# CloudEngineHub/FairyGen

Hardware: AMD Instinct MI355X
Metric: decoded frames/sec (sec/clip in config), Wan2.2-TI2V-5B 704x1280x121 @ 5 steps (higher is better)
Workload: dtype bf16

## Files before the change

fairygen_amd/csrc/dit_elementwise.hip:

```cpp
#include "common.h"
#include "rmsnorm_rope_row.h"

#ifndef FG_ROW_MIN_WAVES
#define FG_ROW_MIN_WAVES 4
#endif
#define FG_ROW_BOUNDS __launch_bounds__(256, FG_ROW_MIN_WAVES)

namespace {

__device__ __forceinline__ void row_moments(const Row& r, int C, int lane, float eps, float& mean, float& rstd) {
    const int nvec = C >> 3;
    float s = 0.f;
#pragma unroll
    for (int i = 0; i < kMaxVec; ++i)
#pragma unroll
        for (int j = 0; j < 8; ++j) s += r.v[i][j];
    mean = wave_sum(s) / (float)C;
    float q = 0.f;
#pragma unroll
    for (int i = 0; i < kMaxVec; ++i) {
        if (lane + i * 64 < nvec) {
#pragma unroll
            for (int j = 0; j < 8; ++j) {
                const float d = r.v[i][j] - mean;
                q += d * d;
            }
        }
    }
    const float var = wave_sum(q) / (float)C;
    rstd = 1.0f / sqrtf(var + eps);
}

__device__ __forceinline__ int64_t mod_row(int64_t row, int64_t mod_rows, int64_t first_rows) {
    return mod_rows == 1 ? 0 : (mod_rows == 2 ? (row < first_rows ? 0 : 1) : row);
}

template <int MODE>
__device__ __forceinline__ void norm_store(const Row& r, int C, int lane, float eps, const bf16* p0, const bf16* p1,
                                           bf16* out) {
    const int nvec = C >> 3;
    float mean, rstd;
    row_moments(r, C, lane, eps, mean, rstd);
#pragma unroll
    for (int i = 0; i < kMaxVec; ++i) {
        const int vi = lane + i * 64;
        if (vi < nvec) {
            const bf16x8 a = ld8(p0 + (int64_t)vi * 8);
            const bf16x8 b = ld8(p1 + (int64_t)vi * 8);
            float o[8];
#pragma unroll
            for (int j = 0; j < 8; ++j) {
                const float n = (r.v[i][j] - mean) * rstd;
                if (MODE == 0) {
                    const float y = rbf(n);
                    const float s1 = rbf(1.0f + (float)b[j]);
                    o[j] = rbf(y * s1) + (float)a[j];
                } else {
                    o[j] = n * (float)a[j] + (float)b[j];
                }
            }
            st8(out + (int64_t)vi * 8, o);
        }
    }
}

__device__ __forceinline__ uint32_t cvt2_fp8(float a, float b) {
    return (uint32_t)__builtin_amdgcn_cvt_pk_fp8_f32(a, b, 0, false) & 0xffffu;
}

template <int MODE, bool DUAL = false>
__device__ __forceinline__ void norm_store_fp8(Row& r, int C, int lane, float eps, const bf16* p0, const bf16* p1,
                                               uint8_t* out8, float* scale_out, float fp8_max, bf16* out16 = nullptr) {
    const int nvec = C >> 3;
    float mean, rstd;
    row_moments(r, C, lane, eps, mean, rstd);
    float amax = 0.f;
#pragma unroll
    for (int i = 0; i < kMaxVec; ++i) {
        const int vi = lane + i * 64;
        if (vi < nvec) {
            const bf16x8 a = ld8(p0 + (int64_t)vi * 8);
            const bf16x8 b = ld8(p1 + (int64_t)vi * 8);
#pragma unroll
            for (int j = 0; j < 8; ++j) {
                const float n = (r.v[i][j] - mean) * rstd;
                float o;
                if (MODE == 0) {
                    const float y = rbf(n);
                    const float s1 = rbf(1.0f + (float)b[j]);
                    o = rbf(y * s1) + (float)a[j];
                } else {
                    o = n * (float)a[j] + (float)b[j];
                }
                r.v[i][j] = rbf(o);
                amax = fmaxf(amax, fabsf(r.v[i][j]));
            }
            if (DUAL) st8(out16 + (int64_t)vi * 8, r.v[i]);
        }
    }
    amax = wave_max(amax);
    const float sc = fmaxf(rbf(amax / fp8_max), 1.0f);
    const float denom = sc + 1e-8f;
    if (lane == 0) *scale_out = sc;
#pragma unroll
    for (int i = 0; i < kMaxVec; ++i) {
        const int vi = lane + i * 64;
        if (vi < nvec) {
            u32x2 w;
// ... 26 lines not shown
    const int64_t row = (int64_t)blockIdx.x * kRowsPerBlock + (threadIdx.x >> 6);
    if (row >= rows) return;
    Row r;
    load_row(x + row * C, C, lane, r);
    const int64_t m = MODE == 0 ? mod_row(row, mod_rows, first_rows) : 0;
    norm_store_fp8<MODE, true>(r, C, lane, eps, p0 + m * mod_ld, p1 + m * mod_ld, out8 + row * C, scale_out + row, fp8_max, out + row * C);
}

__global__ FG_ROW_BOUNDS void ln_modulate_kernel(const bf16* __restrict__ x, const bf16* __restrict__ shift,
                                                          const bf16* __restrict__ scale, bf16* __restrict__ out,
                                                          int64_t rows, int C, float eps, int64_t mod_rows,
                                                          int64_t first_rows, int64_t mod_ld) {
    const int lane = threadIdx.x & 63;
    const int64_t row = (int64_t)blockIdx.x * kRowsPerBlock + (threadIdx.x >> 6);
    if (row >= rows) return;
    Row r;
    load_row(x + row * C, C, lane, r);
    const int64_t m = mod_row(row, mod_rows, first_rows);
    norm_store<0>(r, C, lane, eps, shift + m * mod_ld, scale + m * mod_ld, out + row * C);
}

__global__ FG_ROW_BOUNDS void ln_affine_kernel(const bf16* __restrict__ x, const bf16* __restrict__ w,
                                                        const bf16* __restrict__ b, bf16* __restrict__ out,
                                                        int64_t rows, int C, float eps) {
    const int lane = threadIdx.x & 63;
    const int64_t row = (int64_t)blockIdx.x * kRowsPerBlock + (threadIdx.x >> 6);
    if (row >= rows) return;
    Row r;
    load_row(x + row * C, C, lane, r);
    norm_store<1>(r, C, lane, eps, w, b, out + row * C);
}

template <int MODE>
__global__ FG_ROW_BOUNDS void residual_kernel(const bf16* __restrict__ x, const bf16* __restrict__ y,
                                                       const bf16* __restrict__ gate, bf16* __restrict__ x_out,
                                                       const bf16* __restrict__ p0, const bf16* __restrict__ p1,
                                                       bf16* __restrict__ norm_out, int64_t rows, int C, float eps,
                                                       int64_t mod_rows, int64_t first_rows, int64_t mod_ld,
                                                       uint8_t* __restrict__ norm_fp8 = nullptr, float* __restrict__ norm_scale = nullptr,
                                                       float fp8_max = 0.f) {
    const int lane = threadIdx.x & 63;
    const int64_t row = (int64_t)blockIdx.x * kRowsPerBlock + (threadIdx.x >> 6);
    if (row >= rows) return;
    const int nvec = C >> 3;
    const int64_t m = mod_row(row, mod_rows, first_rows);
    Row r;
#pragma unroll
    for (int i = 0; i < kMaxVec; ++i) {
        const int vi = lane + i * 64;
        if (vi < nvec) {
            const bf16x8 xv = ld8(x + row * C + (int64_t)vi * 8);
            const bf16x8 yv = ld8(y + row * C + (int64_t)vi * 8);
            if (gate != nullptr) {
                const bf16x8 gv = ld8(gate + m * mod_ld + (int64_t)vi * 8);
#pragma unroll
                for (int j = 0; j < 8; ++j) r.v[i][j] = rbf((float)xv[j] + rbf((float)gv[j] * (float)yv[j]));
            } else {
#pragma unroll
                for (int j = 0; j < 8; ++j) r.v[i][j] = rbf((float)xv[j] + (float)yv[j]);
            }
            st8(x_out + row * C + (int64_t)vi * 8, r.v[i]);
        } else {
#pragma unroll
            for (int j = 0; j < 8; ++j) r.v[i][j] = 0.f;
        }
    }
    if (norm_fp8 != nullptr) {
        if (MODE == 0) norm_store_fp8<0>(r, C, lane, eps, p0 + m * mod_ld, p1 + m * mod_ld, norm_fp8 + row * C, norm_scale + row, fp8_max);
        if (MODE == 1) norm_store_fp8<1>(r, C, lane, eps, p0, p1, norm_fp8 + row * C, norm_scale + row, fp8_max);
        return;
    }
    if (MODE == 0) norm_store<0>(r, C, lane, eps, p0 + m * mod_ld, p1 + m * mod_ld, norm_out + row * C);
    if (MODE == 1) norm_store<1>(r, C, lane, eps, p0, p1, norm_out + row * C);
}

template <bool F32TAB, bool PLAIN = false>
__global__ FG_ROW_BOUNDS void rmsnorm_rope_kernel(const bf16* __restrict__ x, int64_t ldx,
                                                           const bf16* __restrict__ w, const void* __restrict__ ctv,
                                                           const void* __restrict__ stv, bf16* __restrict__ out,
                                                           int64_t rows, int C, int head_dim, float eps, int group_cols,
                                                           int64_t out_group_stride, int64_t out_ld) {
    const int lane = threadIdx.x & 63;
    const int64_t row = (int64_t)blockIdx.x * kRowsPerBlock + (threadIdx.x >> 6);
    if (row >= rows) return;
    Row r;
    load_row(x + row * ldx, C, lane, r);
    const int nvec = C >> 3;
    const RopeRow rr = rope_begin<F32TAB, PLAIN>(r, ctv, row, C, head_dim, eps, lane);
#pragma unroll
    for (int i = 0; i < kMaxVec; ++i) {
        const int vi = lane + i * 64;
        if (vi < nvec) {
            float o[8];
            rope_vec<F32TAB, PLAIN>(rr, r.v[i], ld8(w + (int64_t)vi * 8), ctv, stv, row, head_dim, vi, o);
            const int col = vi * 8, g = PLAIN ? 0 : col / group_cols;
            st8(out + g * out_group_stride + row * out_ld + (col - g * group_cols), o);
        }
    }
}

__global__ __launch_bounds__(256) void copy_groups_kernel(const bf16* __restrict__ src, int64_t sgs, int64_t sld,
                                                          bf16* __restrict__ dst, int64_t dgs, int64_t dld, int groups,
                                                          int64_t rows, int vec_per_row) {
    const int64_t total = (int64_t)groups * rows * vec_per_row;
    for (int64_t i = (int64_t)blockIdx.x * blockDim.x + threadIdx.x; i < total; i += (int64_t)gridDim.x * blockDim.x) {
        const int64_t rg = i / vec_per_row;
        const int v = (int)(i - rg * vec_per_row);
        const int64_t r = rg / groups;
        const int g = (int)(rg - r * groups);
        *reinterpret_cast<u32x4*>(dst + g * dgs + r * dld + v * 8) =
            *reinterpret_cast<const u32x4*>(src + g * sgs + r * sld + v * 8);
    }
}


template <int KIND>
__global__ __launch_bounds__(256) void act_kernel(const bf16* __restrict__ x, bf16* __restrict__ out, int64_t nvec) {
    for (int64_t i = (int64_t)blockIdx.x * blockDim.x + threadIdx.x; i < nvec; i += (int64_t)gridDim.x * blockDim.x) {
        const bf16x8 v = ld8(x + i * 8);
        float o[8];
#pragma unroll
        for (int j = 0; j < 8; ++j) o[j] = KIND == 0 ? silu_f((float)v[j]) : gelu_tanh_f((float)v[j]);
        st8(out + i * 8, o);
    }
}

__device__ __forceinline__ float cfg_euler_one(float lat, float p, float ng, bool has_nega, float cfg, float dsigma) {
    const float pred = has_nega ? rbf(ng + rbf(cfg * rbf(p - ng))) : p;
    return rbf(lat + rbf(pred * dsigma));
// ... 22 lines not shown
        if (first != nullptr) {
            int64_t ch = (i * 8) / frame_stride, r = i * 8 - ch * frame_stride;
            if (r < first_n || r + 7 >= frame_stride) {
#pragma unroll
                for (int j = 0; j < 8; ++j) {
                    if (r < first_n) o[j] = (float)first[ch * first_n + r];
                    if (++r == frame_stride) { r = 0; ++ch; }
                }
            }
        }
        st8(out + i * 8, o);
    }
    for (int64_t i = nvec * 8 + tid; i < n; i += nthreads) {
        float o = cfg_euler_one((float)lat[i], (float)posi[i], has_nega ? (float)nega[i] : 0.0f, has_nega, cfg, dsigma);
        if (first != nullptr) {
            const int64_t ch = i / frame_stride, r = i - ch * frame_stride;
            if (r < first_n) o = (float)first[ch * first_n + r];
        }
        out[i] = (bf16)o;
    }
}

inline int check_rows(const char* fn, int64_t rows, int C, int64_t mod_rows, int64_t first_rows) {
    FG_CHECK_ARG(rows >= 0 && C > 0 && (C % 8) == 0 && C <= kMaxVec * 512, "%s: need C %% 8 == 0 and C <= %d (got rows=%lld C=%d)",
                 fn, kMaxVec * 512, (long long)rows, C);
    FG_CHECK_ARG(mod_rows == 1 || mod_rows == 2 || mod_rows == rows, "%s: mod_rows must be 1, 2 or rows (got %lld)", fn,
                 (long long)mod_rows);
    FG_CHECK_ARG(first_rows >= 0 && first_rows <= rows, "%s: first_rows out of range", fn);
    return FG_OK;
}

inline dim3 row_grid(int64_t rows) { return dim3((unsigned)((rows + kRowsPerBlock - 1) / kRowsPerBlock)); }

}

extern "C" {

int fg_ln_modulate_bf16(const void* x, const void* shift, const void* scale, void* out, int64_t rows, int C, float eps,
                        int64_t mod_rows, int64_t first_rows, int64_t mod_ld, fg_stream_t stream) {
    if (int e = check_rows("fg_ln_modulate_bf16", rows, C, mod_rows, first_rows)) return e;
    FG_CHECK_ARG(x && shift && scale && out, "fg_ln_modulate_bf16: null pointer");
    FG_CHECK_ARG(FG_ALIGNED16(x) && FG_ALIGNED16(shift) && FG_ALIGNED16(scale) && FG_ALIGNED16(out) && mod_ld % 8 == 0,
                 "fg_ln_modulate_bf16: pointers / mod_ld must be 16-byte aligned");
    if (rows == 0) return FG_OK;
    hipLaunchKernelGGL(ln_modulate_kernel, row_grid(rows), dim3(256), 0, (hipStream_t)stream, (const bf16*)x,
                       (const bf16*)shift, (const bf16*)scale, (bf16*)out, rows, C, eps, mod_rows, first_rows, mod_ld);
    return fg_launch_status("fg_ln_modulate_bf16");
}

int fg_ln_modulate_fp8_bf16(const void* x, const void* shift, const void* scale, void* out_fp8, float* out_scale, int64_t rows, int C,
                            float eps, int64_t mod_rows, int64_t first_rows, int64_t mod_ld, float fp8_max, fg_stream_t stream) {
    if (int e = check_rows("fg_ln_modulate_fp8_bf16", rows, C, mod_rows, first_rows)) return e;
    FG_CHECK_ARG(x && shift && scale && out_fp8 && out_scale, "fg_ln_modulate_fp8_bf16: null pointer");
    FG_CHECK_ARG(FG_ALIGNED16(x) && FG_ALIGNED16(shift) && FG_ALIGNED16(scale) && (((uintptr_t)out_fp8) & 7) == 0 && mod_ld % 8 == 0 &&
                     fp8_max > 0.f,
                 "fg_ln_modulate_fp8_bf16: pointers / mod_ld must be 16-byte aligned (out_fp8: 8), fp8_max positive");
    if (rows == 0) return FG_OK;
    hipLaunchKernelGGL(ln_modulate_fp8_kernel, row_grid(rows), dim3(256), 0, (hipStream_t)stream, (const bf16*)x, (const bf16*)shift,
                       (const bf16*)scale, (uint8_t*)out_fp8, out_scale, rows, C, eps, mod_rows, first_rows, mod_ld, fp8_max);
    return fg_launch_status("fg_ln_modulate_fp8_bf16");
}

int fg_ln_modulate_dual_bf16(const void* x, const void* shift, const void* scale, void* out, void* out_fp8, float* out_scale,
                             int64_t rows, int C, float eps, int64_t mod_rows, int64_t first_rows, int64_t mod_ld, float fp8_max,
                             fg_stream_t stream) {
    if (int e = check_rows("fg_ln_modulate_dual_bf16", rows, C, mod_rows, first_rows)) return e;
    FG_CHECK_ARG(x && shift && scale && out && out_fp8 && out_scale, "fg_ln_modulate_dual_bf16: null pointer");
    FG_CHECK_ARG(FG_ALIGNED16(x) && FG_ALIGNED16(shift) && FG_ALIGNED16(scale) && FG_ALIGNED16(out) && (((uintptr_t)out_fp8) & 7) == 0 &&
                     mod_ld % 8 == 0 && fp8_max > 0.f,
                 "fg_ln_modulate_dual_bf16: pointers / mod_ld must be 16-byte aligned (out_fp8: 8), fp8_max positive");
    if (rows == 0) return FG_OK;
    hipLaunchKernelGGL(ln_dual_kernel<0>, row_grid(rows), dim3(256), 0, (hipStream_t)stream, (const bf16*)x, (const bf16*)shift,
                       (const bf16*)scale, (bf16*)out, (uint8_t*)out_fp8, out_scale, rows, C, eps, mod_rows, first_rows, mod_ld, fp8_max);
    return fg_launch_status("fg_ln_modulate_dual_bf16");
}

int fg_ln_affine_dual_bf16(const void* x, const void* w, const void* b, void* out, void* out_fp8, float* out_scale, int64_t rows, int C,
                           float eps, float fp8_max, fg_stream_t stream) {
    if (int e = check_rows("fg_ln_affine_dual_bf16", rows, C, 1, 0)) return e;
    FG_CHECK_ARG(x && w && b && out && out_fp8 && out_scale, "fg_ln_affine_dual_bf16: null pointer");
// ... 1 lines not shown
                     fp8_max > 0.f,
                 "fg_ln_affine_dual_bf16: pointers must be 16-byte aligned (out_fp8: 8), fp8_max positive");
    if (rows == 0) return FG_OK;
    hipLaunchKernelGGL(ln_dual_kernel<1>, row_grid(rows), dim3(256), 0, (hipStream_t)stream, (const bf16*)x, (const bf16*)w,
                       (const bf16*)b, (bf16*)out, (uint8_t*)out_fp8, out_scale, rows, C, eps, (int64_t)1, (int64_t)0, (int64_t)0, fp8_max);
    return fg_launch_status("fg_ln_affine_dual_bf16");
}

int fg_residual_ln_fp8_bf16(const void* x, const void* y, const void* gate, void* x_out, const void* p0, const void* p1,
                            void* norm_fp8, float* norm_scale, int mode, int64_t rows, int C, float eps, int64_t mod_rows,
                            int64_t first_rows, int64_t mod_ld, float fp8_max, fg_stream_t stream) {
    FG_CHECK_ARG(mode == 0 || mode == 1, "fg_residual_ln_fp8_bf16: mode must be 0 (modulate) or 1 (affine)");
    const bool need_mod = gate != nullptr || mode == 0;
    if (int e = check_rows("fg_residual_ln_fp8_bf16", rows, C, need_mod ? mod_rows : 1, need_mod ? first_rows : 0)) return e;
    FG_CHECK_ARG(x && y && x_out && p0 && p1 && norm_fp8 && norm_scale, "fg_residual_ln_fp8_bf16: null pointer");
    FG_CHECK_ARG(FG_ALIGNED16(x) && FG_ALIGNED16(y) && FG_ALIGNED16(gate) && FG_ALIGNED16(x_out) && FG_ALIGNED16(p0) &&
                     FG_ALIGNED16(p1) && (((uintptr_t)norm_fp8) & 7) == 0 && mod_ld % 8 == 0 && fp8_max > 0.f,
                 "fg_residual_ln_fp8_bf16: pointers / mod_ld must be 16-byte aligned (norm_fp8: 8), fp8_max positive");
    if (rows == 0) return FG_OK;
    if (!need_mod) { mod_rows = 1; first_rows = 0; }
    if (mode == 0)
        hipLaunchKernelGGL(residual_kernel<0>, row_grid(rows), dim3(256), 0, (hipStream_t)stream, (const bf16*)x,
                           (const bf16*)y, (const bf16*)gate, (bf16*)x_out, (const bf16*)p0, (const bf16*)p1,
                           (bf16*)nullptr, rows, C, eps, mod_rows, first_rows, mod_ld, (uint8_t*)norm_fp8, norm_scale, fp8_max);
    else
        hipLaunchKernelGGL(residual_kernel<1>, row_grid(rows), dim3(256), 0, (hipStream_t)stream, (const bf16*)x,
                           (const bf16*)y, (const bf16*)gate, (bf16*)x_out, (const bf16*)p0, (const bf16*)p1,
                           (bf16*)nullptr, rows, C, eps, mod_rows, first_rows, mod_ld, (uint8_t*)norm_fp8, norm_scale, fp8_max);
    return fg_launch_status("fg_residual_ln_fp8_bf16");
}

int fg_ln_affine_bf16(const void* x, const void* w, const void* b, void* out, int64_t rows, int C, float eps,
                      fg_stream_t stream) {
    if (int e = check_rows("fg_ln_affine_bf16", rows, C, 1, 0)) return e;
    FG_CHECK_ARG(x && w && b && out, "fg_ln_affine_bf16: null pointer");
    FG_CHECK_ARG(FG_ALIGNED16(x) && FG_ALIGNED16(w) && FG_ALIGNED16(b) && FG_ALIGNED16(out),
                 "fg_ln_affine_bf16: pointers must be 16-byte aligned");
    if (rows == 0) return FG_OK;
    hipLaunchKernelGGL(ln_affine_kernel, row_grid(rows), dim3(256), 0, (hipStream_t)stream, (const bf16*)x, (const bf16*)w,
                       (const bf16*)b, (bf16*)out, rows, C, eps);
    return fg_launch_status("fg_ln_affine_bf16");
}

int fg_gate_residual_bf16(const void* x, const void* y, const void* gate, void* out, int64_t rows, int C, int64_t mod_rows,
                          int64_t first_rows, int64_t mod_ld, fg_stream_t stream) {
    if (int e = check_rows("fg_gate_residual_bf16", rows, C, gate ? mod_rows : 1, gate ? first_rows : 0)) return e;
    FG_CHECK_ARG(x && y && out, "fg_gate_residual_bf16: null pointer");
    FG_CHECK_ARG(FG_ALIGNED16(x) && FG_ALIGNED16(y) && FG_ALIGNED16(gate) && FG_ALIGNED16(out) && mod_ld % 8 == 0,
                 "fg_gate_residual_bf16: pointers / mod_ld must be 16-byte aligned");
    if (rows == 0) return FG_OK;
    hipLaunchKernelGGL(residual_kernel<-1>, row_grid(rows), dim3(256), 0, (hipStream_t)stream, (const bf16*)x,
                       (const bf16*)y, (const bf16*)gate, (bf16*)out, (const bf16*)nullptr, (const bf16*)nullptr,
                       (bf16*)nullptr, rows, C, 0.f, gate ? mod_rows : 1, gate ? first_rows : 0, mod_ld);
    return fg_launch_status("fg_gate_residual_bf16");
}

int fg_residual_ln_bf16(const void* x, const void* y, const void* gate, void* x_out, const void* p0, const void* p1,
                        void* norm_out, int mode, int64_t rows, int C, float eps, int64_t mod_rows, int64_t first_rows,
                        int64_t mod_ld, fg_stream_t stream) {
    FG_CHECK_ARG(mode == 0 || mode == 1, "fg_residual_ln_bf16: mode must be 0 (modulate) or 1 (affine)");
    const bool need_mod = gate != nullptr || mode == 0;
    if (int e = check_rows("fg_residual_ln_bf16", rows, C, need_mod ? mod_rows : 1, need_mod ? first_rows : 0)) return e;
    FG_CHECK_ARG(x && y && x_out && p0 && p1 && norm_out, "fg_residual_ln_bf16: null pointer");
    FG_CHECK_ARG(FG_ALIGNED16(x) && FG_ALIGNED16(y) && FG_ALIGNED16(gate) && FG_ALIGNED16(x_out) && FG_ALIGNED16(p0) &&
                     FG_ALIGNED16(p1) && FG_ALIGNED16(norm_out) && mod_ld % 8 == 0,
                 "fg_residual_ln_bf16: pointers / mod_ld must be 16-byte aligned");
    if (rows == 0) return FG_OK;
    if (!need_mod) { mod_rows = 1; first_rows = 0; }
    if (mode == 0)
        hipLaunchKernelGGL(residual_kernel<0>, row_grid(rows), dim3(256), 0, (hipStream_t)stream, (const bf16*)x,
                           (const bf16*)y, (const bf16*)gate, (bf16*)x_out, (const bf16*)p0, (const bf16*)p1,
                           (bf16*)norm_out, rows, C, eps, mod_rows, first_rows, mod_ld);
    else
        hipLaunchKernelGGL(residual_kernel<1>, row_grid(rows), dim3(256), 0, (hipStream_t)stream, (const bf16*)x,
                           (const bf16*)y, (const bf16*)gate, (bf16*)x_out, (const bf16*)p0, (const bf16*)p1,
                           (bf16*)norm_out, rows, C, eps, mod_rows, first_rows, mod_ld);
    return fg_launch_status("fg_residual_ln_bf16");
}

int fg_rmsnorm_rope_bf16(const void* x, int64_t ldx, const void* weight, const void* cos_tab, const void* sin_tab,
                         int table_f32, void* out, int64_t rows, int C, int num_heads, float eps, fg_stream_t stream) {
    if (int e = check_rows("fg_rmsnorm_rope_bf16", rows, C, 1, 0)) return e;
    FG_CHECK_ARG(x && weight && out, "fg_rmsnorm_rope_bf16: null pointer");
    FG_CHECK_ARG(table_f32 ? (cos_tab != nullptr && sin_tab == nullptr) : ((cos_tab == nullptr) == (sin_tab == nullptr)),
                 "fg_rmsnorm_rope_bf16: fp64 mode takes both tables or neither, fp32 mode ONE interleaved table in cos_tab");
    FG_CHECK_ARG(num_heads > 0 && C % num_heads == 0 && (C / num_heads) % 8 == 0,
                 "fg_rmsnorm_rope_bf16: head_dim must be a multiple of 8");
    FG_CHECK_ARG(ldx >= C && ldx % 8 == 0 && FG_ALIGNED16(x) && FG_ALIGNED16(weight) && FG_ALIGNED16(out) &&
                     FG_ALIGNED16(cos_tab) && FG_ALIGNED16(sin_tab),
                 "fg_rmsnorm_rope_bf16: pointers / ldx must be 16-byte aligned");
    if (rows == 0) return FG_OK;
    const int hd = C / num_heads;
    const bool plain = (hd & (hd - 1)) == 0;
#define FG_ROPE_LAUNCH(TAB, PL)                                                                                                  \
    hipLaunchKernelGGL((rmsnorm_rope_kernel<TAB, PL>), row_grid(rows), dim3(256), 0, (hipStream_t)stream, (const bf16*)x, ldx,    \
                       (const bf16*)weight, cos_tab, sin_tab, (bf16*)out, rows, C, hd, eps, C, (int64_t)0, (int64_t)C)
    if (table_f32) { if (plain) FG_ROPE_LAUNCH(true, true); else FG_ROPE_LAUNCH(true, false); }
    else { if (plain) FG_ROPE_LAUNCH(false, true); else FG_ROPE_LAUNCH(false, false); }
#undef FG_ROPE_LAUNCH
    return fg_launch_status("fg_rmsnorm_rope_bf16");
}

int fg_rmsnorm_rope_grouped_bf16(const void* x, int64_t ldx, const void* weight, const void* cos_tab,
                                 const void* sin_tab, int table_f32, void* out, int64_t rows, int C, int num_heads, float eps,
                                 int group_cols, int64_t out_group_stride, int64_t out_ld, fg_stream_t stream) {
    if (int e = check_rows("fg_rmsnorm_rope_grouped_bf16", rows, C, 1, 0)) return e;
    FG_CHECK_ARG(x && weight && out, "fg_rmsnorm_rope_grouped_bf16: null pointer");
    FG_CHECK_ARG(table_f32 ? (cos_tab != nullptr && sin_tab == nullptr) : ((cos_tab == nullptr) == (sin_tab == nullptr)),
                 "fg_rmsnorm_rope_grouped_bf16: fp64 mode takes both tables or neither, fp32 mode ONE interleaved table in cos_tab");
    FG_CHECK_ARG(num_heads > 0 && C % num_heads == 0 && (C / num_heads) % 8 == 0,
                 "fg_rmsnorm_rope_grouped_bf16: head_dim must be a multiple of 8");
    FG_CHECK_ARG(group_cols > 0 && group_cols % 8 == 0 && C % group_cols == 0 && out_ld >= group_cols && out_ld % 8 == 0 &&
                     out_group_stride % 8 == 0 && out_group_stride >= 0,
                 "fg_rmsnorm_rope_grouped_bf16: group_cols must divide C; group_cols, out_ld, out_group_stride multiples of 8");
    FG_CHECK_ARG(ldx >= C && ldx % 8 == 0 && FG_ALIGNED16(x) && FG_ALIGNED16(weight) && FG_ALIGNED16(out) &&
                     FG_ALIGNED16(cos_tab) && FG_ALIGNED16(sin_tab),
                 "fg_rmsnorm_rope_grouped_bf16: pointers / ldx must be 16-byte aligned");
    if (rows == 0) return FG_OK;
    if (table_f32)
        hipLaunchKernelGGL((rmsnorm_rope_kernel<true, false>), row_grid(rows), dim3(256), 0, (hipStream_t)stream, (const bf16*)x, ldx,
                           (const bf16*)weight, cos_tab, sin_tab, (bf16*)out, rows, C, C / num_heads, eps, group_cols,
                           out_group_stride, out_ld);
    else
        hipLaunchKernelGGL((rmsnorm_rope_kernel<false, false>), row_grid(rows), dim3(256), 0, (hipStream_t)stream, (const bf16*)x, ldx,
                           (const bf16*)weight, cos_tab, sin_tab, (bf16*)out, rows, C, C / num_heads, eps, group_cols,
                           out_group_stride, out_ld);
    return fg_launch_status("fg_rmsnorm_rope_grouped_bf16");
}

int fg_copy_groups_bf16(const void* src, int64_t src_group_stride, int64_t src_ld, void* dst, int64_t dst_group_stride,
                        int64_t dst_ld, int groups, int64_t rows, int cols, fg_stream_t stream) {
    FG_CHECK_ARG(src && dst, "fg_copy_groups_bf16: null pointer");
    FG_CHECK_ARG(groups > 0 && rows >= 0 && cols > 0 && cols % 8 == 0, "fg_copy_groups_bf16: cols must be a positive multiple of 8");
// ... 55 lines not shown
```

fairygen_amd/csrc/rmsnorm_rope_row.h:

```cpp
#pragma once
#include "common.h"

namespace {

constexpr int kMaxVec = 8;
constexpr int kRowsPerBlock = 4;

template <int NV>
struct RowT {
    float v[NV][8];
};
typedef RowT<kMaxVec> Row;

template <int NV>
__device__ __forceinline__ void load_row(const bf16* p, int C, int lane, RowT<NV>& r) {
    const int nvec = C >> 3;
#pragma unroll
    for (int i = 0; i < NV; ++i) {
        const int vi = lane + i * 64;
        if (vi < nvec) {
            bf16x8 t = *reinterpret_cast<const bf16x8*>(p + (int64_t)vi * 8);
#pragma unroll
            for (int j = 0; j < 8; ++j) r.v[i][j] = (float)t[j];
        } else {
#pragma unroll
            for (int j = 0; j < 8; ++j) r.v[i][j] = 0.f;
        }
    }
}

__device__ __forceinline__ bf16x8 ld8(const bf16* p) { return *reinterpret_cast<const bf16x8*>(p); }
__device__ __forceinline__ void st8(bf16* p, const float* f) {
    bf16x8 t;
#pragma unroll
    for (int j = 0; j < 8; ++j) t[j] = (bf16)f[j];
    *reinterpret_cast<bf16x8*>(p) = t;
}

struct RopeRow {
    float rinv;
    bool hoist;
    f32x4 h0, h1;
};

template <bool F32TAB, bool PLAIN, int NV>
__device__ __forceinline__ RopeRow rope_begin(const RowT<NV>& r, const void* ctv, int64_t row, int C, int head_dim, float eps, int lane) {
    RopeRow c;
    float q = 0.f;
#pragma unroll
    for (int i = 0; i < NV; ++i)
#pragma unroll
        for (int j = 0; j < 8; ++j) q += r.v[i][j] * r.v[i][j];
    const float ms = wave_sum(q) / (float)C;
    c.rinv = 1.0f / sqrtf(ms + eps);
    const int half = head_dim >> 1;
    c.hoist = F32TAB && ctv != nullptr && (512 % head_dim) == 0;
    c.h0 = f32x4{0.f, 0.f, 0.f, 0.f};
    c.h1 = f32x4{0.f, 0.f, 0.f, 0.f};
    if (c.hoist) {
        const int d_lane = PLAIN ? ((lane * 8) & (head_dim - 1)) : ((lane * 8) % head_dim);
        const f32x4* tp = reinterpret_cast<const f32x4*>(static_cast<const float*>(ctv) + (row * half + (d_lane >> 1)) * 2);
// ... 44 lines not shown
```

fairygen_amd/hip.py:

```python
import ctypes
import os

import torch

_LIB_PATH = os.environ.get("FAIRYGEN_HIP_LIB") or os.path.join(os.path.dirname(os.path.abspath(__file__)), "libfairygen_hip.so")
_lib = None

ABI_VERSION = 8
QK8_ABI_VERSION = 1
QK8F_ABI_VERSION = 1

_i64, _i32, _f32, _vp = ctypes.c_int64, ctypes.c_int, ctypes.c_float, ctypes.c_void_p

_SIGNATURES = {
    "fg_ln_modulate_bf16": [_vp, _vp, _vp, _vp, _i64, _i32, _f32, _i64, _i64, _i64, _vp],
    "fg_ln_affine_bf16": [_vp, _vp, _vp, _vp, _i64, _i32, _f32, _vp],
    "fg_ln_modulate_fp8_bf16": [_vp, _vp, _vp, _vp, _vp, _i64, _i32, _f32, _i64, _i64, _i64, _f32, _vp],
    "fg_residual_ln_fp8_bf16": [_vp, _vp, _vp, _vp, _vp, _vp, _vp, _vp, _i32, _i64, _i32, _f32, _i64, _i64, _i64, _f32, _vp],
    "fg_ln_modulate_dual_bf16": [_vp, _vp, _vp, _vp, _vp, _vp, _i64, _i32, _f32, _i64, _i64, _i64, _f32, _vp],
    "fg_ln_affine_dual_bf16": [_vp, _vp, _vp, _vp, _vp, _vp, _i64, _i32, _f32, _f32, _vp],
    "fg_gate_residual_bf16": [_vp, _vp, _vp, _vp, _i64, _i32, _i64, _i64, _i64, _vp],
    "fg_residual_ln_bf16": [_vp, _vp, _vp, _vp, _vp, _vp, _vp, _i32, _i64, _i32, _f32, _i64, _i64, _i64, _vp],
    "fg_rmsnorm_rope_bf16": [_vp, _i64, _vp, _vp, _vp, _i32, _vp, _i64, _i32, _i32, _f32, _vp],
    "fg_rmsnorm_rope_grouped_bf16": [_vp, _i64, _vp, _vp, _vp, _i32, _vp, _i64, _i32, _i32, _f32, _i32, _i64, _i64, _vp],
# ... 53 lines not shown
    "fg_attn_fwd_pv8_bf16": [_vp, _vp, _vp, _vp, _vp, _vp, _vp, _i64, _i64, _i32, _i32, _f32, _vp, _i64, _vp],
}
_PV8_QUERIES = {
    "fg_attn_pv8_version": (_i32, []),
    "fg_attn_pv8_scratch_bytes": (_i64, [_i64, _i32]),
}
PV8_SYMBOLS = sorted(list(_PV8_SIGNATURES) + list(_PV8_QUERIES))
PV8_KEY_ORDER = tuple(32 * ((p >> 4) & 1) + 8 * ((p & 15) >> 2) + 4 * (p >> 5) + (p & 3) for p in range(64))
PV8_LOG2_C, PV8_DEFER_LOG2 = 5, 3

SHARD8_ABI_VERSION = 1
_SHARD8_SIGNATURES = {
    "fg_attn_shard8_stats": [_vp, _i64, _vp, _i64, _vp, _i64, _vp, _i64, _i64, _i32, _i32, _vp],
    "fg_attn_shard8_quant": [_vp, _i64, _i32, _i64, _vp, _i64, _vp, _i64, _vp, _vp, _vp, _vp, _vp, _i64, _i32, _i32, _vp],
    "fg_attn_shard8_vt": [_vp, _vp, _i64, _i32, _i32, _vp],
}
_SHARD8_QUERIES = {
    "fg_attn_shard8_version": (_i32, []),
    "fg_attn_shard8_record_bytes": (_i64, [_i32]),
    "fg_attn_shard8_scratch_bytes": (_i64, [_i64, _i32]),
}
SHARD8_SYMBOLS = sorted(list(_SHARD8_SIGNATURES) + list(_SHARD8_QUERIES))

CROSS8_ABI_VERSION = 1
_CROSS8_SIGNATURES = {
    "fg_attn_fwd_cross8_bf16": [_vp, _vp, _vp, _vp, _vp, _vp, _vp, _i64, _i64, _i32, _i32, _f32, _vp],
}
_CROSS8_QUERIES = {
    "fg_attn_cross8_version": (_i32, []),
    "fg_attn_cross8_max_kv": (_i64, []),
}
CROSS8_SYMBOLS = sorted(list(_CROSS8_SIGNATURES) + list(_CROSS8_QUERIES))


class HipLibraryError(RuntimeError):
    pass


def library_path():
    return _LIB_PATH


def load():
    global _lib
    if _lib is not None:
        return _lib
    if not os.path.exists(_LIB_PATH):
        raise HipLibraryError(
            f"{_LIB_PATH} not found: build it with `make -C fairygen_amd/csrc` (or __graft_entry__.build()). "
            "fairygen_amd has no CPU / PyTorch fallback for its kernels.")
    lib = ctypes.CDLL(_LIB_PATH)
    for name, argtypes in list(_SIGNATURES.items()) + list(_PV8_SIGNATURES.items()) + list(_SHARD8_SIGNATURES.items()) + \
            list(_CROSS8_SIGNATURES.items()):
        getattr(lib, name).restype, getattr(lib, name).argtypes = _i32, argtypes
    for name, (restype, argtypes) in list(_QUERIES.items()) + list(_PV8_QUERIES.items()) + list(_SHARD8_QUERIES.items()) + \
            list(_CROSS8_QUERIES.items()):
        getattr(lib, name).restype, getattr(lib, name).argtypes = restype, argtypes
    for name, expected, what in (("fg_version", ABI_VERSION, ""), ("fg_attn_qk8_version", QK8_ABI_VERSION, " (e4m3 Q K^T extension)"),
                                 ("fg_attn_qk8_fused_version", QK8F_ABI_VERSION, " (fused e4m3 producers)"),
                                 ("fg_attn_pv8_version", PV8_ABI_VERSION, " (e4m3 P V extension)"),
                                 ("fg_attn_shard8_version", SHARD8_ABI_VERSION, " (e4m3 operands of a token shard)"),
                                 ("fg_attn_cross8_version", CROSS8_ABI_VERSION, " (e4m3 cross-attention, K8 / V8^T in LDS)")):
        if getattr(lib, name)() != expected:
            raise HipLibraryError(f"ABI mismatch{what}: library {getattr(lib, name)()} != binding {expected}")
    _lib = lib
    return lib


def _call(name, *args):
    lib = load()
    rc = getattr(lib, name)(*args)
    if rc != 0:
        raise HipLibraryError(f"{name} failed ({rc}): {lib.fg_last_error().decode()}")


def _stream(t):
    return ctypes.c_void_p(torch.cuda.current_stream(t.device).cuda_stream)


def _dev(t, name, dtype=torch.bfloat16):
    if not isinstance(t, torch.Tensor) or t.device.type != "cuda":
        raise HipLibraryError(f"{name}: expected a tensor on a HIP device, got {getattr(t, 'device', type(t))} "
                              "(no CPU fallback)")
    if t.dtype != dtype:
        raise HipLibraryError(f"{name}: expected dtype {dtype}, got {t.dtype}")
    return t


def _ptr(t):
    return ctypes.c_void_p(t.data_ptr()) if t is not None else ctypes.c_void_p(0)


def _rows(t, name):
    _dev(t, name)
    if not t.is_contiguous():
# ... 845 lines not shown
```

Before: 15.54.

## Add C=3072 specialized row kernels with row-walk prefetch for LN and RMSNorm-RoPE

```diff
diff --git a/fairygen_amd/csrc/dit_elementwise.hip b/fairygen_amd/csrc/dit_elementwise.hip
--- a/fairygen_amd/csrc/dit_elementwise.hip
+++ b/fairygen_amd/csrc/dit_elementwise.hip
@@ -1,5 +1,6 @@
 #include "common.h"
 #include "rmsnorm_rope_row.h"
+#include "../../include/fairygen_hip_rowref.h"
 
 #ifndef FG_ROW_MIN_WAVES
 #define FG_ROW_MIN_WAVES 4
@@ -8,18 +9,19 @@
 
 namespace {
 
-__device__ __forceinline__ void row_moments(const Row& r, int C, int lane, float eps, float& mean, float& rstd) {
+template <int NV, bool FULL>
+__device__ __forceinline__ void row_moments(const RowT<NV>& r, int C, int lane, float eps, float& mean, float& rstd) {
     const int nvec = C >> 3;
     float s = 0.f;
 #pragma unroll
-    for (int i = 0; i < kMaxVec; ++i)
+    for (int i = 0; i < NV; ++i)
 #pragma unroll
         for (int j = 0; j < 8; ++j) s += r.v[i][j];
     mean = wave_sum(s) / (float)C;
     float q = 0.f;
 #pragma unroll
-    for (int i = 0; i < kMaxVec; ++i) {
-        if (lane + i * 64 < nvec) {
+    for (int i = 0; i < NV; ++i) {
+        if (FULL || lane + i * 64 < nvec) {
 #pragma unroll
             for (int j = 0; j < 8; ++j) {
                 const float d = r.v[i][j] - mean;
@@ -33,6 +35,21 @@
 
 __device__ __forceinline__ int64_t mod_row(int64_t row, int64_t mod_rows, int64_t first_rows) {
     return mod_rows == 1 ? 0 : (mod_rows == 2 ? (row < first_rows ? 0 : 1) : row);
+}
+
+template <int MODE>
+__device__ __forceinline__ void norm_vec(const float* rv, float mean, float rstd, const bf16x8 a, const bf16x8 b, float* o) {
+#pragma unroll
+    for (int j = 0; j < 8; ++j) {
+        const float n = (rv[j] - mean) * rstd;
+        if (MODE == 0) {
+            const float y = rbf(n);
+            const float s1 = rbf(1.0f + (float)b[j]);
+            o[j] = rbf(y * s1) + (float)a[j];
+        } else {
+            o[j] = n * (float)a[j] + (float)b[j];
+        }
+    }
 }
 
 template <int MODE>
@@ -40,27 +57,36 @@
                                            bf16* out) {
     const int nvec = C >> 3;
     float mean, rstd;
-    row_moments(r, C, lane, eps, mean, rstd);
+    row_moments<kMaxVec, false>(r, C, lane, eps, mean, rstd);
 #pragma unroll
     for (int i = 0; i < kMaxVec; ++i) {
         const int vi = lane + i * 64;
         if (vi < nvec) {
-            const bf16x8 a = ld8(p0 + (int64_t)vi * 8);
-            const bf16x8 b = ld8(p1 + (int64_t)vi * 8);
             float o[8];
-#pragma unroll
-            for (int j = 0; j < 8; ++j) {
-                const float n = (r.v[i][j] - mean) * rstd;
-                if (MODE == 0) {
-                    const float y = rbf(n);
-                    const float s1 = rbf(1.0f + (float)b[j]);
-                    o[j] = rbf(y * s1) + (float)a[j];
-                } else {
-                    o[j] = n * (float)a[j] + (float)b[j];
-                }
-            }
+            norm_vec<MODE>(r.v[i], mean, rstd, ld8(p0 + (int64_t)vi * 8), ld8(p1 + (int64_t)vi * 8), o);
             st8(out + (int64_t)vi * 8, o);
         }
+    }
+}
+
+template <int MODE>
+__device__ __forceinline__ void norm_store_fast(const RowT<kFastVec>& r, int lane, float eps, const bf16* p0, const bf16* p1, bf16* out) {
+    bf16x8 a = ld8(p0 + (int64_t)lane * 8), b = ld8(p1 + (int64_t)lane * 8);
+    float mean, rstd;
+    row_moments<kFastVec, true>(r, kFastC, lane, eps, mean, rstd);
+#pragma unroll
+    for (int i = 0; i < kFastVec; ++i) {
+        const int vi = lane + i * 64;
+        bf16x8 an = a, bn = b;
+        if (i + 1 < kFastVec) {
+            an = ld8(p0 + (int64_t)(vi + 64) * 8);
+            bn = ld8(p1 + (int64_t)(vi + 64) * 8);
+        }
+        float o[8];
+        norm_vec<MODE>(r.v[i], mean, rstd, a, b, o);
+        st8(out + (int64_t)vi * 8, o);
+        a = an;
+        b = bn;
     }
 }
 
@@ -73,7 +99,7 @@
                                                uint8_t* out8, float* scale_out, float fp8_max, bf16* out16 = nullptr) {
     const int nvec = C >> 3;
     float mean, rstd;
-    row_moments(r, C, lane, eps, mean, rstd);
+    row_moments<kMaxVec, false>(r, C, lane, eps, mean, rstd);
     float amax = 0.f;
 #pragma unroll
     for (int i = 0; i < kMaxVec; ++i) {
@@ -166,6 +192,24 @@
 }
 
 template <int MODE>
+__global__ FG_ROW_BOUNDS void ln_rows_fast_kernel(const bf16* x, const bf16* p0, const bf16* p1, bf16* out, int64_t rows, float eps, int64_t mod_rows,
+                                                  int64_t first_rows, int64_t mod_ld) {
+    const int lane = threadIdx.x & 63;
+    const int64_t step = (int64_t)gridDim.x * kRowsPerBlock;
+    int64_t row = (int64_t)blockIdx.x * kRowsPerBlock + __builtin_amdgcn_readfirstlane((int)(threadIdx.x >> 6));
+    if (row >= rows) return;
+    RawRowT<kFastVec> next;
+    load_raw(x + row * kFastC, lane, next);
+    for (; row < rows; row += step) {
+        RowT<kFastVec> r;
+        widen(next, r);
+        if (row + step < rows) load_raw(x + (row + step) * kFastC, lane, next);
+        const int64_t m = MODE == 0 ? mod_row(row, mod_rows, first_rows) : 0;
+        norm_store_fast<MODE>(r, lane, eps, p0 + m * mod_ld, p1 + m * mod_ld, out + row * kFastC);
+    }
+}
+
+template <int MODE>
 __global__ FG_ROW_BOUNDS void residual_kernel(const bf16* __restrict__ x, const bf16* __restrict__ y,
                                                        const bf16* __restrict__ gate, bf16* __restrict__ x_out,
                                                        const bf16* __restrict__ p0, const bf16* __restrict__ p1,
@@ -229,6 +273,35 @@
             rope_vec<F32TAB, PLAIN>(rr, r.v[i], ld8(w + (int64_t)vi * 8), ctv, stv, row, head_dim, vi, o);
             const int col = vi * 8, g = PLAIN ? 0 : col / group_cols;
             st8(out + g * out_group_stride + row * out_ld + (col - g * group_cols), o);
+        }
+    }
+}
+
+template <bool F32TAB>
+__global__ FG_ROW_BOUNDS void rmsnorm_rope_fast_kernel(const bf16* x, int64_t ldx, const bf16* w, const void* ctv, const void* stv,
+                                                       bf16* out, int64_t rows, float eps) {
+    constexpr int kHead = 128;
+    const int lane = threadIdx.x & 63;
+    const int64_t step = (int64_t)gridDim.x * kRowsPerBlock;
+    int64_t row = (int64_t)blockIdx.x * kRowsPerBlock + __builtin_amdgcn_readfirstlane((int)(threadIdx.x >> 6));
+    if (row >= rows) return;
+    RawRowT<kFastVec> next;
+    load_raw(x + row * ldx, lane, next);
+    for (; row < rows; row += step) {
+        RowT<kFastVec> r;
+        widen(next, r);
+        if (row + step < rows) load_raw(x + (row + step) * ldx, lane, next);
+        bf16x8 wv = ld8(w + (int64_t)lane * 8);
+        const RopeRow rr = rope_begin<F32TAB, true>(r, ctv, row, kFastC, kHead, eps, lane);
+#pragma unroll
+        for (int i = 0; i < kFastVec; ++i) {
+            const int vi = lane + i * 64;
+            bf16x8 wn = wv;
+            if (i + 1 < kFastVec) wn = ld8(w + (int64_t)(vi + 64) * 8);
+            float o[8];
+            rope_vec<F32TAB, true>(rr, r.v[i], wv, ctv, stv, row, kHead, vi, o);
+            st8(out + row * kFastC + (int64_t)vi * 8, o);
+            wv = wn;
         }
     }
 }
@@ -317,20 +390,98 @@
 
 inline dim3 row_grid(int64_t rows) { return dim3((unsigned)((rows + kRowsPerBlock - 1) / kRowsPerBlock)); }
 
+constexpr int kRowWalk = 3;
+inline dim3 row_walk_grid(int64_t rows) {
+    const int64_t per_block = (int64_t)kRowsPerBlock * kRowWalk;
+    return dim3((unsigned)((rows + per_block - 1) / per_block));
+}
+
+int ln_modulate_impl(const char* fn, bool fast, const void* x, const void* shift, const void* scale, void* out, int64_t rows, int C,
+                     float eps, int64_t mod_rows, int64_t first_rows, int64_t mod_ld, fg_stream_t stream) {
+    if (int e = check_rows(fn, rows, C, mod_rows, first_rows)) return e;
+    FG_CHECK_ARG(x && shift && scale && out, "%s: null pointer", fn);
+    FG_CHECK_ARG(FG_ALIGNED16(x) && FG_ALIGNED16(shift) && FG_ALIGNED16(scale) && FG_ALIGNED16(out) && mod_ld % 8 == 0,
+                 "%s: pointers / mod_ld must be 16-byte aligned", fn);
+    if (rows == 0) return FG_OK;
+    if (fast && C == kFastC)
+        hipLaunchKernelGGL(ln_rows_fast_kernel<0>, row_walk_grid(rows), dim3(256), 0, (hipStream_t)stream, (const bf16*)x,
+                           (const bf16*)shift, (const bf16*)scale, (bf16*)out, rows, eps, mod_rows, first_rows, mod_ld);
+    else
+        hipLaunchKernelGGL(ln_modulate_kernel, row_grid(rows), dim3(256), 0, (hipStream_t)stream, (const bf16*)x,
+                           (const bf16*)shift, (const bf16*)scale, (bf16*)out, rows, C, eps, mod_rows, first_rows, mod_ld);
+    return fg_launch_status(fn);
+}
+
+int ln_affine_impl(const char* fn, bool fast, const void* x, const void* w, const void* b, void* out, int64_t rows, int C, float eps,
+                   fg_stream_t stream) {
+    if (int e = check_rows(fn, rows, C, 1, 0)) return e;
+    FG_CHECK_ARG(x && w && b && out, "%s: null pointer", fn);
+    FG_CHECK_ARG(FG_ALIGNED16(x) && FG_ALIGNED16(w) && FG_ALIGNED16(b) && FG_ALIGNED16(out), "%s: pointers must be 16-byte aligned", fn);
+    if (rows == 0) return FG_OK;
+    if (fast && C == kFastC)
+        hipLaunchKernelGGL(ln_rows_fast_kernel<1>, row_walk_grid(rows), dim3(256), 0, (hipStream_t)stream, (const bf16*)x, (const bf16*)w,
+                           (const bf16*)b, (bf16*)out, rows, eps, (int64_t)1, (int64_t)0, (int64_t)0);
+    else
+        hipLaunchKernelGGL(ln_affine_kernel, row_grid(rows), dim3(256), 0, (hipStream_t)stream, (const bf16*)x, (const bf16*)w,
+                           (const bf16*)b, (bf16*)out, rows, C, eps);
+    return fg_launch_status(fn);
+}
+
+int rmsnorm_rope_impl(const char* fn, bool fast, const void* x, int64_t ldx, const void* weight, const void* cos_tab, const void* sin_tab,
+                      int table_f32, void* out, int64_t rows, int C, int num_heads, float eps, fg_stream_t stream) {
+    if (int e = check_rows(fn, rows, C, 1, 0)) return e;
+    FG_CHECK_ARG(x && weight && out, "%s: null pointer", fn);
+    FG_CHECK_ARG(table_f32 ? (cos_tab != nullptr && sin_tab == nullptr) : ((cos_tab == nullptr) == (sin_tab == nullptr)),
+                 "%s: fp64 mode takes both tables or neither, fp32 mode ONE interleaved table in cos_tab", fn);
+    FG_CHECK_ARG(num_heads > 0 && C % num_heads == 0 && (C / num_heads) % 8 == 0, "%s: head_dim must be a multiple of 8", fn);
+    FG_CHECK_ARG(ldx >= C && ldx % 8 == 0 && FG_ALIGNED16(x) && FG_ALIGNED16(weight) && FG_ALIGNED16(out) &&
+                     FG_ALIGNED16(cos_tab) && FG_ALIGNED16(sin_tab),
+                 "%s: pointers / ldx must be 16-byte aligned", fn);
+    if (rows == 0) return FG_OK;
+    const int hd = C / num_heads;
+    const bool plain = (hd & (hd - 1)) == 0;
+    if (fast && C == kFastC && hd == 128) {
+        if (table_f32)
+            hipLaunchKernelGGL(rmsnorm_rope_fast_kernel<true>, row_walk_grid(rows), dim3(256), 0, (hipStream_t)stream, (const bf16*)x, ldx,
+                               (const bf16*)weight, cos_tab, sin_tab, (bf16*)out, rows, eps);
+        else
+            hipLaunchKernelGGL(rmsnorm_rope_fast_kernel<false>, row_walk_grid(rows), dim3(256), 0, (hipStream_t)stream, (const bf16*)x, ldx,
+                               (const bf16*)weight, cos_tab, sin_tab, (bf16*)out, rows, eps);
+        return fg_launch_status(fn);
+    }
+#define FG_ROPE_LAUNCH(TAB, PL)                                                                                                  \
+    hipLaunchKernelGGL((rmsnorm_rope_kernel<TAB, PL>), row_grid(rows), dim3(256), 0, (hipStream_t)stream, (const bf16*)x, ldx,    \
+                       (const bf16*)weight, cos_tab, sin_tab, (bf16*)out, rows, C, hd, eps, C, (int64_t)0, (int64_t)C)
+    if (table_f32) { if (plain) FG_ROPE_LAUNCH(true, true); else FG_ROPE_LAUNCH(true, false); }
+    else { if (plain) FG_ROPE_LAUNCH(false, true); else FG_ROPE_LAUNCH(false, false); }
+#undef FG_ROPE_LAUNCH
+    return fg_launch_status(fn);
+}
+
 }
 
 extern "C" {
 
 int fg_ln_modulate_bf16(const void* x, const void* shift, const void* scale, void* out, int64_t rows, int C, float eps,
                         int64_t mod_rows, int64_t first_rows, int64_t mod_ld, fg_stream_t stream) {
-    if (int e = check_rows("fg_ln_modulate_bf16", rows, C, mod_rows, first_rows)) return e;
-    FG_CHECK_ARG(x && shift && scale && out, "fg_ln_modulate_bf16: null pointer");
-    FG_CHECK_ARG(FG_ALIGNED16(x) && FG_ALIGNED16(shift) && FG_ALIGNED16(scale) && FG_ALIGNED16(out) && mod_ld % 8 == 0,
-                 "fg_ln_modulate_bf16: pointers / mod_ld must be 16-byte aligned");
-    if (rows == 0) return FG_OK;
-    hipLaunchKernelGGL(ln_modulate_kernel, row_grid(rows), dim3(256), 0, (hipStream_t)stream, (const bf16*)x,
-                       (const bf16*)shift, (const bf16*)scale, (bf16*)out, rows, C, eps, mod_rows, first_rows, mod_ld);
-    return fg_launch_status("fg_ln_modulate_bf16");
+    return ln_modulate_impl("fg_ln_modulate_bf16", true, x, shift, scale, out, rows, C, eps, mod_rows, first_rows, mod_ld, stream);
+}
+
+int fg_row_ref_version(void) { return 1; }
+
+int fg_ln_modulate_ref_bf16(const void* x, const void* shift, const void* scale, void* out, int64_t rows, int C, float eps,
+                            int64_t mod_rows, int64_t first_rows, int64_t mod_ld, fg_stream_t stream) {
+    return ln_modulate_impl("fg_ln_modulate_ref_bf16", false, x, shift, scale, out, rows, C, eps, mod_rows, first_rows, mod_ld, stream);
+}
+
+int fg_ln_affine_ref_bf16(const void* x, const void* w, const void* b, void* out, int64_t rows, int C, float eps, fg_stream_t stream) {
+    return ln_affine_impl("fg_ln_affine_ref_bf16", false, x, w, b, out, rows, C, eps, stream);
+}
+
+int fg_rmsnorm_rope_ref_bf16(const void* x, int64_t ldx, const void* weight, const void* cos_tab, const void* sin_tab, int table_f32,
+                             void* out, int64_t rows, int C, int num_heads, float eps, fg_stream_t stream) {
+    return rmsnorm_rope_impl("fg_rmsnorm_rope_ref_bf16", false, x, ldx, weight, cos_tab, sin_tab, table_f32, out, rows, C, num_heads, eps,
+                             stream);
 }
 
 int fg_ln_modulate_fp8_bf16(const void* x, const void* shift, const void* scale, void* out_fp8, float* out_scale, int64_t rows, int C,
@@ -398,14 +549,7 @@
 
 int fg_ln_affine_bf16(const void* x, const void* w, const void* b, void* out, int64_t rows, int C, float eps,
                       fg_stream_t stream) {
-    if (int e = check_rows("fg_ln_affine_bf16", rows, C, 1, 0)) return e;
-    FG_CHECK_ARG(x && w && b && out, "fg_ln_affine_bf16: null pointer");
-    FG_CHECK_ARG(FG_ALIGNED16(x) && FG_ALIGNED16(w) && FG_ALIGNED16(b) && FG_ALIGNED16(out),
-                 "fg_ln_affine_bf16: pointers must be 16-byte aligned");
-    if (rows == 0) return FG_OK;
-    hipLaunchKernelGGL(ln_affine_kernel, row_grid(rows), dim3(256), 0, (hipStream_t)stream, (const bf16*)x, (const bf16*)w,
-                       (const bf16*)b, (bf16*)out, rows, C, eps);
-    return fg_launch_status("fg_ln_affine_bf16");
+    return ln_affine_impl("fg_ln_affine_bf16", true, x, w, b, out, rows, C, eps, stream);
 }
 
 int fg_gate_residual_bf16(const void* x, const void* y, const void* gate, void* out, int64_t rows, int C, int64_t mod_rows,
@@ -446,25 +590,7 @@
 
 int fg_rmsnorm_rope_bf16(const void* x, int64_t ldx, const void* weight, const void* cos_tab, const void* sin_tab,
                          int table_f32, void* out, int64_t rows, int C, int num_heads, float eps, fg_stream_t stream) {
-    if (int e = check_rows("fg_rmsnorm_rope_bf16", rows, C, 1, 0)) return e;
-    FG_CHECK_ARG(x && weight && out, "fg_rmsnorm_rope_bf16: null pointer");
-    FG_CHECK_ARG(table_f32 ? (cos_tab != nullptr && sin_tab == nullptr) : ((cos_tab == nullptr) == (sin_tab == nullptr)),
-                 "fg_rmsnorm_rope_bf16: fp64 mode takes both tables or neither, fp32 mode ONE interleaved table in cos_tab");
-    FG_CHECK_ARG(num_heads > 0 && C % num_heads == 0 && (C / num_heads) % 8 == 0,
-                 "fg_rmsnorm_rope_bf16: head_dim must be a multiple of 8");
-    FG_CHECK_ARG(ldx >= C && ldx % 8 == 0 && FG_ALIGNED16(x) && FG_ALIGNED16(weight) && FG_ALIGNED16(out) &&
-                     FG_ALIGNED16(cos_tab) && FG_ALIGNED16(sin_tab),
-                 "fg_rmsnorm_rope_bf16: pointers / ldx must be 16-byte aligned");
-    if (rows == 0) return FG_OK;
-    const int hd = C / num_heads;
-    const bool plain = (hd & (hd - 1)) == 0;
-#define FG_ROPE_LAUNCH(TAB, PL)                                                                                                  \
-    hipLaunchKernelGGL((rmsnorm_rope_kernel<TAB, PL>), row_grid(rows), dim3(256), 0, (hipStream_t)stream, (const bf16*)x, ldx,    \
-                       (const bf16*)weight, cos_tab, sin_tab, (bf16*)out, rows, C, hd, eps, C, (int64_t)0, (int64_t)C)
-    if (table_f32) { if (plain) FG_ROPE_LAUNCH(true, true); else FG_ROPE_LAUNCH(true, false); }
-    else { if (plain) FG_ROPE_LAUNCH(false, true); else FG_ROPE_LAUNCH(false, false); }
-#undef FG_ROPE_LAUNCH
-    return fg_launch_status("fg_rmsnorm_rope_bf16");
+    return rmsnorm_rope_impl("fg_rmsnorm_rope_bf16", true, x, ldx, weight, cos_tab, sin_tab, table_f32, out, rows, C, num_heads, eps, stream);
 }
 
 int fg_rmsnorm_rope_grouped_bf16(const void* x, int64_t ldx, const void* weight, const void* cos_tab,
diff --git a/fairygen_amd/csrc/rmsnorm_rope_row.h b/fairygen_amd/csrc/rmsnorm_rope_row.h
--- a/fairygen_amd/csrc/rmsnorm_rope_row.h
+++ b/fairygen_amd/csrc/rmsnorm_rope_row.h
@@ -27,6 +27,28 @@
             for (int j = 0; j < 8; ++j) r.v[i][j] = 0.f;
         }
     }
+}
+
+constexpr int kFastVec = 6;
+constexpr int kFastC = kFastVec * 512;
+
+template <int NV>
+struct RawRowT {
+    bf16x8 v[NV];
+};
+
+template <int NV>
+__device__ __forceinline__ void load_raw(const bf16* p, int lane, RawRowT<NV>& t) {
+#pragma unroll
+    for (int i = 0; i < NV; ++i) t.v[i] = *reinterpret_cast<const bf16x8*>(p + (int64_t)(lane + i * 64) * 8);
+}
+
+template <int NV>
+__device__ __forceinline__ void widen(const RawRowT<NV>& t, RowT<NV>& r) {
+#pragma unroll
+    for (int i = 0; i < NV; ++i)
+#pragma unroll
+        for (int j = 0; j < 8; ++j) r.v[i][j] = (float)t.v[i][j];
 }
 
 __device__ __forceinline__ bf16x8 ld8(const bf16* p) { return *reinterpret_cast<const bf16x8*>(p); }
diff --git a/fairygen_amd/hip.py b/fairygen_amd/hip.py
--- a/fairygen_amd/hip.py
+++ b/fairygen_amd/hip.py
@@ -109,6 +109,17 @@
 }
 CROSS8_SYMBOLS = sorted(list(_CROSS8_SIGNATURES) + list(_CROSS8_QUERIES))
 
+ROWREF_ABI_VERSION = 1
+_ROWREF_SIGNATURES = {
+    "fg_ln_modulate_ref_bf16": [_vp, _vp, _vp, _vp, _i64, _i32, _f32, _i64, _i64, _i64, _vp],
+    "fg_ln_affine_ref_bf16": [_vp, _vp, _vp, _vp, _i64, _i32, _f32, _vp],
+    "fg_rmsnorm_rope_ref_bf16": [_vp, _i64, _vp, _vp, _vp, _i32, _vp, _i64, _i32, _i32, _f32, _vp],
+}
+_ROWREF_QUERIES = {
+    "fg_row_ref_version": (_i32, []),
+}
+ROWREF_SYMBOLS = sorted(list(_ROWREF_SIGNATURES) + list(_ROWREF_QUERIES))
+
 
 class HipLibraryError(RuntimeError):
     pass
@@ -128,16 +139,17 @@
             "fairygen_amd has no CPU / PyTorch fallback for its kernels.")
     lib = ctypes.CDLL(_LIB_PATH)
     for name, argtypes in list(_SIGNATURES.items()) + list(_PV8_SIGNATURES.items()) + list(_SHARD8_SIGNATURES.items()) + \
-            list(_CROSS8_SIGNATURES.items()):
+            list(_CROSS8_SIGNATURES.items()) + list(_ROWREF_SIGNATURES.items()):
         getattr(lib, name).restype, getattr(lib, name).argtypes = _i32, argtypes
     for name, (restype, argtypes) in list(_QUERIES.items()) + list(_PV8_QUERIES.items()) + list(_SHARD8_QUERIES.items()) + \
-            list(_CROSS8_QUERIES.items()):
+            list(_CROSS8_QUERIES.items()) + list(_ROWREF_QUERIES.items()):
         getattr(lib, name).restype, getattr(lib, name).argtypes = restype, argtypes
     for name, expected, what in (("fg_version", ABI_VERSION, ""), ("fg_attn_qk8_version", QK8_ABI_VERSION, " (e4m3 Q K^T extension)"),
                                  ("fg_attn_qk8_fused_version", QK8F_ABI_VERSION, " (fused e4m3 producers)"),
                                  ("fg_attn_pv8_version", PV8_ABI_VERSION, " (e4m3 P V extension)"),
                                  ("fg_attn_shard8_version", SHARD8_ABI_VERSION, " (e4m3 operands of a token shard)"),
-                                 ("fg_attn_cross8_version", CROSS8_ABI_VERSION, " (e4m3 cross-attention, K8 / V8^T in LDS)")):
+                                 ("fg_attn_cross8_version", CROSS8_ABI_VERSION, " (e4m3 cross-attention, K8 / V8^T in LDS)"),
+                                 ("fg_row_ref_version", ROWREF_ABI_VERSION, " (generic row kernels as a reference)")):
         if getattr(lib, name)() != expected:
             raise HipLibraryError(f"ABI mismatch{what}: library {getattr(lib, name)()} != binding {expected}")
     _lib = lib
diff --git a/include/fairygen_hip_rowref.h b/include/fairygen_hip_rowref.h
--- /dev/null
+++ b/include/fairygen_hip_rowref.h
@@ -0,0 +1,23 @@
+#ifndef FAIRYGEN_HIP_ROWREF_H
+#define FAIRYGEN_HIP_ROWREF_H
+
+#include "fairygen_hip.h"
+
+#ifdef __cplusplus
+extern "C" {
+#endif
+
+int fg_row_ref_version(void);
+
+int fg_ln_modulate_ref_bf16(const void* x, const void* shift, const void* scale, void* out, int64_t rows, int C, float eps,
+                            int64_t mod_rows, int64_t first_rows, int64_t mod_ld, fg_stream_t stream);
+
+int fg_ln_affine_ref_bf16(const void* x, const void* w, const void* b, void* out, int64_t rows, int C, float eps, fg_stream_t stream);
+
+int fg_rmsnorm_rope_ref_bf16(const void* x, int64_t ldx, const void* weight, const void* cos_tab, const void* sin_tab, int table_f32,
+                             void* out, int64_t rows, int C, int num_heads, float eps, fg_stream_t stream);
+
+#ifdef __cplusplus
+}
+#endif
+#endif
```

After: 15.59 (median of 6 runs). Within noise of the previous version (+0.3%).
